# WarmCongee/SDUMC

Hardware: AMD Instinct MI355X
Metric: train samples/sec at MOSEI feature shapes (two-stream forward + 6-term loss + backward + Adam) (higher is better)
Workload: dtype f32

## Files before the change

### sdumc_amd/csrc/attn_pool.hip

```cpp
#include <type_traits>

#include "common.h"
#include "p3_loop.h"
#include <cstring>

namespace {

constexpr int D = SDUMC_D;
constexpr int MAXQ = 8;
constexpr int CH = 64;

__device__ __forceinline__ f32x4 ld4(const float* p) { return *reinterpret_cast<const f32x4*>(p); }
__device__ __forceinline__ void st4(float* p, f32x4 v) { *reinterpret_cast<f32x4*>(p) = v; }
__device__ __forceinline__ void stf_dev(float* p, float v) { __hip_atomic_store(p, v, __ATOMIC_RELAXED, __HIP_MEMORY_SCOPE_AGENT); }
__device__ __forceinline__ float ldf_dev(const float* p) { return __hip_atomic_load(p, __ATOMIC_RELAXED, __HIP_MEMORY_SCOPE_AGENT); }
__device__ __forceinline__ void st4_dev(float* p, f32x4 v) {
#pragma unroll
  for (int j = 0; j < 4; ++j) stf_dev(p + j, v[j]);
}
__device__ __forceinline__ f32x4 ld4_dev(const float* p) {
  f32x4 v;
#pragma unroll
  for (int j = 0; j < 4; ++j) v[j] = ldf_dev(p + j);
  return v;
// ... 1284 lines not shown
    }
  };

  constexpr int nk = D / BK;
#pragma unroll
  for (int s = 0; s < NST - 1; ++s) issue(s);
  int buf = 0, ibuf = NST - 1;
  for (int t = 0; t < nk; ++t) {
    if (t + NST - 2 < nk) __builtin_amdgcn_s_waitcnt(waitcnt_vm((NST - 2) * PER));
    else __builtin_amdgcn_s_waitcnt(waitcnt_vm(0));
    __builtin_amdgcn_s_barrier();
    if (t + NST - 1 < nk) issue(ibuf);
    if constexpr (SPLIT) compute_split(lds + buf * STAGE_BYTES);
    else compute(lds + buf * STAGE_BYTES);
    buf = buf + 1 == NST ? 0 : buf + 1;
    ibuf = ibuf + 1 == NST ? 0 : ibuf + 1;
  }
  __syncthreads();

  float* K_s = reinterpret_cast<float*>(lds);
  float* q_s = reinterpret_cast<float*>(lds + TOP_BYTES);
  float* keys_out = const_cast<float*>(p.keys);
#pragma unroll
  for (int i = 0; i < 2; ++i)
#pragma unroll
    for (int j = 0; j < 2; ++j) {
      const int col = wn0 + 32 * j + li;
      const float bv = u.b_in[col];
#pragma unroll
      for (int e = 0; e < 16; ++e) {
        const int row = 32 * i + (e & 3) + 8 * (e >> 2) + 4 * lh;
        const float kv = fast_tanh(acc[i][j][e] + bv);
        K_s[row * UMCA_LDK + col] = kv;
        if (keys_out && t0 + row < T) keys_out[((size_t)v * T + t0 + row) * D + col] = kv;
      }
    }
  __syncthreads();
  attn_fwd_partial_body<false, 1, false, true>(p, static_cast<float*>(p.workspace), nchunk, chunk, v, K_s, q_s, K_s);
#endif
}
template <bool MASK>
__global__ __launch_bounds__(256, 2) void umca_fwd_kernel(const sdumc_umca u, const int nchunk) {
  extern __shared__ __attribute__((aligned(16))) char lds[];
  umca_fwd_body<MASK, false>(u, nchunk, lds);
}
template <bool MASK>
__global__ __launch_bounds__(256, 2) void umca_fwd_split_kernel(const sdumc_umca u, const int nchunk) {
  extern __shared__ __attribute__((aligned(16))) char lds[];
  umca_fwd_body<MASK, true>(u, nchunk, lds);
}

using K3P3Cfg_m = sdumc_p3::PCfg<64, 4, true, 4>;
using K3P3Cfg_n = sdumc_p3::PCfg<64, 4, false, 4>;
static_assert(K3P3Cfg_m::LDS_BYTES <= TOP_BYTES, "the P3 ring lies inside the key tile's memory");
template <bool MASK>
__global__ __launch_bounds__(256, 2) void umca_fwd_p3_kernel(const sdumc_umca u, const int nchunk) {
#if defined(__HIP_DEVICE_COMPILE__)
  using CF = std::conditional_t<MASK, K3P3Cfg_m, K3P3Cfg_n>;
  extern __shared__ __attribute__((aligned(16))) char lds[];
  const sdumc_attnpool& p = u.a;
  const int tid = threadIdx.x, lane = tid & 63;
  const int wave = __builtin_amdgcn_readfirstlane(tid >> 6);
  const int li = lane & 31, lh = lane >> 5;
  const int wn0 = wave * 64;
  const int chunk = blockIdx.x, v = blockIdx.y;
  const int T = p.T, t0 = chunk * CH, vx = v % p.x_samples;
  const __amdgpu_buffer_rsrc_t ra = __builtin_amdgcn_make_buffer_rsrc(const_cast<void*>(u.x_p3), 0,
      (int)min((size_t)p.x_samples * T * D * 6, (size_t)0xFFFFFFF0u), 0x00020000);
  const uint32_t qw = (p.x_drop.width + 3u) >> 2;
  const __amdgpu_buffer_rsrc_t rbits = __builtin_amdgcn_make_buffer_rsrc(const_cast<uint8_t*>(MASK ? p.x_drop.bits : static_cast<const uint8_t*>(u.x_p3)), 0,
      MASK ? (int)min((size_t)p.V * T * qw, (size_t)0xFFFFFFF0u) : 0, 0x00020000);
  f32x16 acc[2][2];
  sdumc_p3::p3_mainloop<CF>(lds, ra, (int64_t)D * 6, [&](int row) { return vx * T + min(t0 + row, T - 1); },
                            rbits, (int)qw, [&](int row) { return v * T + min(t0 + row, T - 1); },
                            static_cast<const char*>(u.w_in_p3f) + (size_t)(wave * 2) * (size_t)((D / 16) * sdumc_p3::FRAG_KT), (size_t)((D / 16) * sdumc_p3::FRAG_KT),
                            0, D / sdumc_p3::BK, acc);
  __syncthreads();
  const float mscale = MASK ? p.x_drop.scale : 1.f;
  float* K_s = reinterpret_cast<float*>(lds);
  float* q_s = reinterpret_cast<float*>(lds + TOP_BYTES);
  float* keys_out = const_cast<float*>(p.keys);
#pragma unroll
  for (int i = 0; i < 2; ++i)
#pragma unroll
    for (int j = 0; j < 2; ++j) {
      const int col = wn0 + 32 * j + li;
      const float bv = u.b_in[col];
#pragma unroll
      for (int e = 0; e < 16; ++e) {
        const int row = 32 * i + (e & 3) + 8 * (e >> 2) + 4 * lh;
        const float kv = fast_tanh(acc[i][j][e] * mscale + bv);
        K_s[row * UMCA_LDK + col] = kv;
        if (keys_out && t0 + row < T) keys_out[((size_t)v * T + t0 + row) * D + col] = kv;
      }
    }
  __syncthreads();
  attn_fwd_partial_body<false, 1, false, true>(p, static_cast<float*>(p.workspace), nchunk, chunk, v, K_s, q_s, K_s);
#endif
}

}

static inline uint32_t qw_of(const sdumc_dropout& d) { return (d.width + 3u) >> 2; }
extern "C" int sdumc_umca_fwd(const sdumc_umca* up, void* stream) {
  if (!up) return SDUMC_EINVAL;
  sdumc_umca u = *up;
  const sdumc_attnpool& p = u.a;
  if (p.V <= 0 || p.T <= 0 || p.nq < 1 || p.nq > MAXQ || p.x_samples <= 0) return SDUMC_EINVAL;
  if ((p.dim != 0 && p.dim != D) || p.bf16 || p.tickets) return SDUMC_EINVAL;
  if (!p.x || !p.q || !p.attn || !p.pooled || !p.out || !u.w_in || !u.b_in) return SDUMC_EINVAL;
  if (p.x_drop.enabled && !p.x_drop.bits) return SDUMC_EINVAL;
  if ((p.T + CH - 1) / CH > 4096) return SDUMC_EINVAL;
  if (!p.workspace || p.workspace_bytes < sdumc_attnpool_fwd_workspace_bytes_dim(p.V, p.T, p.nq, D)) return SDUMC_ENOMEM;
  static sdumc_dev_once attr;
  if (sdumc_once_per_device(attr, [] {
        return sdumc_set_dyn_lds(&sdumc_k3::umca_fwd_kernel<true>, sdumc_k3::LDS_BYTES) && sdumc_set_dyn_lds(&sdumc_k3::umca_fwd_kernel<false>, sdumc_k3::LDS_BYTES) &&
               sdumc_set_dyn_lds(&sdumc_k3::umca_fwd_split_kernel<true>, sdumc_k3::LDS_BYTES) && sdumc_set_dyn_lds(&sdumc_k3::umca_fwd_split_kernel<false>, sdumc_k3::LDS_BYTES);
      }) != SDUMC_OK)
    return SDUMC_ELAUNCH;
  hipStream_t st = as_stream(stream);
  const int nchunk = (p.T + CH - 1) / CH;
  const dim3 grid(nchunk, p.V), blk(256);
  if (u.x_p3 && u.w_in_p3f) {
    if (!sdumc_split_on_(SDUMC_SPLIT_UMCA)) return SDUMC_EINVAL;
    if ((reinterpret_cast<uintptr_t>(u.x_p3) | reinterpret_cast<uintptr_t>(u.w_in_p3f)) & 15) return SDUMC_EINVAL;
    if (p.x_drop.enabled && (qw_of(p.x_drop) & 3)) return SDUMC_EINVAL;
    static sdumc_dev_once attr_p3;
    if (sdumc_once_per_device(attr_p3, [] {
          return sdumc_set_dyn_lds(&sdumc_k3::umca_fwd_p3_kernel<true>, sdumc_k3::LDS_BYTES) && sdumc_set_dyn_lds(&sdumc_k3::umca_fwd_p3_kernel<false>, sdumc_k3::LDS_BYTES);
// ... 23 lines not shown
```

### sdumc_amd/csrc/gemm_p3.hip

```cpp
#include <algorithm>
#include <cstdlib>

#include "p3_loop.h"

namespace sdumc_p3 {

struct Args {
  sdumc_gemm_p3 g;
  int nsplit, kchunk;
};

template <class CF, int MAPPED = 0>
__global__ __launch_bounds__(CF::NTHR, CF::NW == 4 ? 2 : 1) void gemm_p3_nt_kernel(const Args a) {
#if defined(__HIP_DEVICE_COMPILE__)
  constexpr int BM = CF::BM, TM = CF::TM, TN = CF::TN;
  constexpr bool MASK = CF::MASK;
  const sdumc_gemm_p3& g = a.g;
  extern __shared__ __attribute__((aligned(16))) char lds[];
  const int tid = threadIdx.x, lane = tid & 63;
  const int wave = __builtin_amdgcn_readfirstlane(tid >> 6);
  const int li = lane & 31, lh = lane >> 5;
  const int tiles_n = g.N / BN;
  const int tlin = blockIdx.x;
  const int tile_m = tlin / tiles_n, tile_n = tlin - tile_m * tiles_n;
  const int ks = blockIdx.y;
  const int m0 = tile_m * BM, n0 = tile_n * BN;
  const int kbeg = ks * a.kchunk, kend = min(g.K, kbeg + a.kchunk);
  const int nk = (kend - kbeg) / BK;

#if defined(SDUMC_P3_DBG) && (SDUMC_P3_DBG & 8)
  const uint64_t dbg_t0 = __builtin_amdgcn_s_memtime(), dbg_r0 = __builtin_amdgcn_s_memrealtime();
#endif
  const bool second = g.A2 != nullptr && m0 >= g.a2_row0;
  const int arow0 = second ? g.a2_row0 : 0;
  const int a_rows = g.a_row_mod > 0 ? g.a_row_mod : (g.A2 ? (second ? g.M - g.a2_row0 : g.a2_row0) : g.M);
  const __amdgpu_buffer_rsrc_t ra = __builtin_amdgcn_make_buffer_rsrc(const_cast<void*>(second ? g.A2 : g.A), 0, (int)min((size_t)a_rows * (size_t)g.lda, (size_t)0xFFFFFFF0u), 0x00020000);
  [[maybe_unused]] const __amdgpu_buffer_rsrc_t rbits = __builtin_amdgcn_make_buffer_rsrc(const_cast<uint8_t*>(MASK ? g.a_bits : static_cast<const uint8_t*>(g.A)), 0,
                                                                        MASK ? (int)min((size_t)g.M * (size_t)g.bits_qw, (size_t)0xFFFFFFF0u) : 0, 0x00020000);

  f32x16 acc[TM][TN];
  uint64_t dbg_r1 = 0;
  const char* bw = static_cast<const char*>(g.B) + (size_t)(tile_n * 8 + wave * TN) * (size_t)g.ldb;
  if constexpr (MAPPED == 2) {
    const char* abase = static_cast<const char*>(second ? g.A2 : g.A);
    const int32_t* amap = second ? g.a2_map : g.a_map;
    p3_mainloop<CF>(lds, ra, g.lda,
                    [&](int row) -> const char* { return abase + (size_t)amap[min(m0 + row, g.M - 1) - arow0] * (size_t)g.lda; },
                    rbits, g.bits_qw, [&](int row) { return min(m0 + row, g.M - 1); }, bw, (size_t)g.ldb, kbeg, nk, acc, &dbg_r1);
  } else if constexpr (MAPPED == 1) {
    const int32_t* amap = second ? g.a2_map : g.a_map;
    const __amdgpu_buffer_rsrc_t rm = __builtin_amdgcn_make_buffer_rsrc(const_cast<void*>(second ? g.A2 : g.A), 0, (int)min((size_t)g.a_map_rows * (size_t)g.lda, (size_t)0xFFFFFFF0u), 0x00020000);
    p3_mainloop<CF>(lds, rm, g.lda, [&](int row) { return amap[min(m0 + row, g.M - 1) - arow0]; },
                    rbits, g.bits_qw, [&](int row) { return min(m0 + row, g.M - 1); }, bw, (size_t)g.ldb, kbeg, nk, acc, &dbg_r1);
  } else {
    p3_mainloop<CF>(lds, ra, g.lda,
                    [&](int row) { int r = min(m0 + row, g.M - 1) - arow0; if (g.a_row_mod > 0) r %= g.a_row_mod; return r; },
                    rbits, g.bits_qw, [&](int row) { return min(m0 + row, g.M - 1); }, bw, (size_t)g.ldb, kbeg, nk, acc, &dbg_r1);
  }
  (void)dbg_r1;
#if defined(SDUMC_P3_DBG) && (SDUMC_P3_DBG & 8)
  const uint64_t dbg_r2 = __builtin_amdgcn_s_memrealtime();
#endif
  const bool to_slab = a.nsplit > 1;
  const float mscale = MASK ? g.a_scale : 1.f;
  constexpr int LDT = CF::LDT, WCOLS = 32 * TN, CPW = WCOLS / 8;
  float* tw = reinterpret_cast<float*>(lds) + wave * 32 * LDT;
  const int colw = n0 + WCOLS * wave;
  float bv[8];
#pragma unroll
  for (int c = 0; c < 8; ++c) bv[c] = (!to_slab && g.bias) ? g.bias[colw + 8 * (lane & (CPW - 1)) + c] : 0.f;
  __syncthreads();
#pragma unroll
  for (int i = 0; i < TM; ++i) {
#pragma unroll
    for (int j = 0; j < TN; ++j)
#pragma unroll
      for (int e = 0; e < 16; ++e) tw[((e & 3) + 8 * (e >> 2) + 4 * lh) * LDT + 32 * j + li] = acc[i][j][e] * mscale;
    __builtin_amdgcn_s_waitcnt(0xC07F);
#pragma unroll
    for (int u = lane; u < 32 * CPW; u += 64) {
      const int r = u / CPW, cq = u % CPW;
      const int row = m0 + 32 * i + r, col = colw + 8 * cq;
      if (row < g.M) {
        const f32x4 a0 = *reinterpret_cast<const f32x4*>(tw + r * LDT + 8 * cq), a1 = *reinterpret_cast<const f32x4*>(tw + r * LDT + 8 * cq + 4);
        float v[8] = {a0[0], a0[1], a0[2], a0[3], a1[0], a1[1], a1[2], a1[3]};
        if (to_slab) {
          float* dst = g.workspace + ((size_t)ks * g.M + row) * g.N + col;
          *reinterpret_cast<f32x4*>(dst) = a0;
          *reinterpret_cast<f32x4*>(dst + 4) = a1;
        } else {
#pragma unroll
          for (int c = 0; c < 8; ++c) {
            float x = v[c] + bv[c];
            if (g.act == SDUMC_ACT_TANH) x = fast_tanh(x);
            else if (g.act == SDUMC_ACT_RELU) x = fmaxf(x, 0.f);
            v[c] = x;
          }
          if (g.C) {
            float* dst = g.C + (size_t)row * g.ldc + col;
            *reinterpret_cast<f32x4*>(dst) = f32x4{v[0], v[1], v[2], v[3]};
            *reinterpret_cast<f32x4*>(dst + 4) = f32x4{v[4], v[5], v[6], v[7]};
          }
          if (g.C_p3) {
            u32x4 pl[3];
            split8(v, pl);
            char* dst = static_cast<char*>(g.C_p3) + (size_t)row * (size_t)g.ldc_p3 + (size_t)(col >> 3) * 48;
            *reinterpret_cast<u32x4*>(dst) = pl[0];
            *reinterpret_cast<u32x4*>(dst + 16) = pl[1];
            *reinterpret_cast<u32x4*>(dst + 32) = pl[2];
          }
// ... 62 lines not shown
    *reinterpret_cast<u32x4*>(dst + 16) = pl[1];
    *reinterpret_cast<u32x4*>(dst + 32) = pl[2];
  }
}

__global__ __launch_bounds__(256) void p3_split_kernel(const float* __restrict__ src, int64_t ld, char* __restrict__ dst, int64_t ldp, int64_t rows,
                                                       int cols) {
  const int cpr = cols >> 3;
  const int64_t total = rows * cpr;
  for (int64_t u = (int64_t)blockIdx.x * 256 + threadIdx.x; u < total; u += (int64_t)gridDim.x * 256) {
    const int64_t row = u / cpr;
    const int c = (int)(u - row * cpr);
    const float* s = src + row * ld + 8 * c;
    const f32x4 a0 = *reinterpret_cast<const f32x4*>(s), a1 = *reinterpret_cast<const f32x4*>(s + 4);
    const float v[8] = {a0[0], a0[1], a0[2], a0[3], a1[0], a1[1], a1[2], a1[3]};
    u32x4 pl[3];
    split8(v, pl);
    char* d = dst + row * ldp + (int64_t)c * 48;
    *reinterpret_cast<u32x4*>(d) = pl[0];
    *reinterpret_cast<u32x4*>(d + 16) = pl[1];
    *reinterpret_cast<u32x4*>(d + 32) = pl[2];
  }
}
__global__ __launch_bounds__(256) void p3_split_frag_kernel(const float* __restrict__ src, int64_t ld, char* __restrict__ dst, int rows, int cols) {
  const int cpr = cols >> 3;
  const int64_t total = (int64_t)rows * cpr;
  for (int64_t u = (int64_t)blockIdx.x * 256 + threadIdx.x; u < total; u += (int64_t)gridDim.x * 256) {
    const int row = (int)(u / cpr), c = (int)(u - (int64_t)row * cpr);
    const float* sp = src + (int64_t)row * ld + 8 * c;
    const f32x4 a0 = *reinterpret_cast<const f32x4*>(sp), a1 = *reinterpret_cast<const f32x4*>(sp + 4);
    const float v[8] = {a0[0], a0[1], a0[2], a0[3], a1[0], a1[1], a1[2], a1[3]};
    u32x4 pl[3];
    split8(v, pl);
    const int rb = row >> 5, li = row & 31, kt = c >> 1, lh = c & 1;
    char* d = dst + ((int64_t)rb * (cols >> 4) + kt) * FRAG_KT + (lh * 32 + li) * 16;
    *reinterpret_cast<u32x4*>(d) = pl[0];
    *reinterpret_cast<u32x4*>(d + 1024) = pl[1];
    *reinterpret_cast<u32x4*>(d + 2048) = pl[2];
  }
}

struct FragList {
  int64_t src_off[12], dst_off[12];
  int32_t rows[12], cols[12];
};
__global__ __launch_bounds__(256) void p3_split_frag_multi_kernel(const float* __restrict__ P, char* __restrict__ dst, const FragList L) {
  const int i = blockIdx.y;
  const int rows = L.rows[i], cols = L.cols[i], cpr = cols >> 3;
  const float* src = P + L.src_off[i];
  char* out = dst + L.dst_off[i];
  const int64_t total = (int64_t)rows * cpr;
  for (int64_t u = (int64_t)blockIdx.x * 256 + threadIdx.x; u < total; u += (int64_t)gridDim.x * 256) {
    const int row = (int)(u / cpr), c = (int)(u - (int64_t)row * cpr);
    const float* sp = src + (int64_t)row * cols + 8 * c;
    const f32x4 a0 = *reinterpret_cast<const f32x4*>(sp), a1 = *reinterpret_cast<const f32x4*>(sp + 4);
    const float v[8] = {a0[0], a0[1], a0[2], a0[3], a1[0], a1[1], a1[2], a1[3]};
    u32x4 pl[3];
    split8(v, pl);
    const int rb = row >> 5, li = row & 31, kt = c >> 1, lh = c & 1;
    char* d = out + ((int64_t)rb * (cols >> 4) + kt) * FRAG_KT + (lh * 32 + li) * 16;
    *reinterpret_cast<u32x4*>(d) = pl[0];
    *reinterpret_cast<u32x4*>(d + 1024) = pl[1];
    *reinterpret_cast<u32x4*>(d + 2048) = pl[2];
  }
}
__global__ __launch_bounds__(256) void p3_join_kernel(const char* __restrict__ src, int64_t ldp, float* __restrict__ dst, int64_t ld, int64_t rows,
                                                      int cols) {
  const int cpr = cols >> 3;
  const int64_t total = rows * cpr;
  for (int64_t u = (int64_t)blockIdx.x * 256 + threadIdx.x; u < total; u += (int64_t)gridDim.x * 256) {
    const int64_t row = u / cpr;
    const int c = (int)(u - row * cpr);
    const char* s = src + row * ldp + (int64_t)c * 48;
    const u32x4 p0 = *reinterpret_cast<const u32x4*>(s), p1 = *reinterpret_cast<const u32x4*>(s + 16), p2 = *reinterpret_cast<const u32x4*>(s + 32);
    float v[8];
#pragma unroll
    for (int d = 0; d < 4; ++d) {
      v[2 * d] = (__uint_as_float(p0[d] << 16) + __uint_as_float(p1[d] << 16)) + __uint_as_float(p2[d] << 16);
      v[2 * d + 1] = (__uint_as_float(p0[d] & 0xFFFF0000u) + __uint_as_float(p1[d] & 0xFFFF0000u)) + __uint_as_float(p2[d] & 0xFFFF0000u);
    }
    float* o = dst + row * ld + 8 * c;
    *reinterpret_cast<f32x4*>(o) = f32x4{v[0], v[1], v[2], v[3]};
    *reinterpret_cast<f32x4*>(o + 4) = f32x4{v[4], v[5], v[6], v[7]};
  }
}

struct Plan {
  int bm, nsplit, kchunk;
};
inline Plan plan(const sdumc_gemm_p3& g, size_t have) {
  const int forced = g.tile_m ? g.tile_m : 64;
  const int tiles_n = g.N / BN;
  Plan best{64, 1, g.K};
// ... 41 lines not shown
  if (!g || g->M <= 0 || g->N <= 0 || g->K <= 0 || (g->K % (4 * sdumc_p3::BK))) return 0;
  const sdumc_p3::Plan p = sdumc_p3::plan(*g, (size_t)-1);
  return p.nsplit > 1 ? (size_t)p.nsplit * g->M * g->N * sizeof(float) : 0;
}

extern "C" int sdumc_gemm_p3_nt(const sdumc_gemm_p3* gp, void* stream) {
  using namespace sdumc_p3;
  if (!gp) return SDUMC_EINVAL;
  const sdumc_gemm_p3& g = *gp;
  if (g.M <= 0 || g.N <= 0 || g.K <= 0 || (g.N % BN) || (g.K % (4 * BK))) return SDUMC_EINVAL;
  if (!g.A || !g.B || (!g.C && !g.C_p3)) return SDUMC_EINVAL;
  if ((reinterpret_cast<uintptr_t>(g.A) | reinterpret_cast<uintptr_t>(g.B) | reinterpret_cast<uintptr_t>(g.C) | reinterpret_cast<uintptr_t>(g.C_p3)) & 15) return SDUMC_EINVAL;
  if (g.lda < 6 * (int64_t)g.K || (g.lda & 15)) return SDUMC_EINVAL;
  if (g.ldb < (int64_t)(g.K / BK) * FRAG_KT || (g.ldb & 15)) return SDUMC_EINVAL;
  if (g.C && ((g.ldc & 3) || g.ldc < g.N)) return SDUMC_EINVAL;
  if (g.C_p3 && ((g.ldc_p3 & 15) || g.ldc_p3 < 6 * (int64_t)g.N)) return SDUMC_EINVAL;
  if (g.tile_m != 0 && g.tile_m != 64 && g.tile_m != 96 && g.tile_m != 128) return SDUMC_EINVAL;
  if (g.A2 && (g.a_row_mod || g.a2_row0 <= 0 || g.a2_row0 >= g.M || (g.a2_row0 % 64) || (g.tile_m && g.a2_row0 % g.tile_m) || (reinterpret_cast<uintptr_t>(g.A2) & 15))) return SDUMC_EINVAL;
  if (g.act != SDUMC_ACT_NONE && g.act != SDUMC_ACT_TANH && g.act != SDUMC_ACT_RELU) return SDUMC_EINVAL;
  const bool mapped = g.a_map != nullptr;
  if (mapped && (g.a_row_mod || g.a_bits || (g.A2 != nullptr) != (g.a2_map != nullptr))) return SDUMC_EINVAL;
  if (!mapped && g.a2_map) return SDUMC_EINVAL;
  const size_t a_bytes = (size_t)(g.a_row_mod > 0 ? g.a_row_mod : (g.A2 ? std::max(g.a2_row0, g.M - g.a2_row0) : g.M)) * (size_t)g.lda;
  if (!mapped && a_bytes >= 0xFFFFFFF0u) return SDUMC_EINVAL;
  const bool mask = g.a_bits != nullptr;
  if (mask && (g.bits_qw < g.K / 4 || (g.bits_qw & 3) || (reinterpret_cast<uintptr_t>(g.a_bits) & 3) || (size_t)g.M * g.bits_qw >= 0xFFFFFFF0u)) return SDUMC_EINVAL;
  const Plan p = plan(g, g.workspace ? g.workspace_bytes : 0);
  if (p.nsplit > 1 && (!g.workspace || (reinterpret_cast<uintptr_t>(g.workspace) & 15))) return SDUMC_ENOMEM;
  hipStream_t st = as_stream(stream);
  const int tok = sdumc_prof_begin_(mask ? 27 : 26, 2.0 * g.M * (double)g.N * g.K, stream);
  int rc;
  const bool map32 = mapped && g.a_map_rows > 0 && (size_t)g.a_map_rows * (size_t)g.lda < 0xFFFFFFF0u;
  if (mapped && g.tile_m) return SDUMC_EINVAL;
  if (map32) rc = launch<PCfg<64, 4, false, 4>, 1>(g, p, st);
  else if (mapped) rc = launch<PCfg<64, 4, false, 4>, 2>(g, p, st);
  else if (!g.tile_m) {
    rc = mask ? launch<PCfg<64, 4, true, 4>>(g, p, st) : launch<PCfg<64, 4, false, 4>>(g, p, st);
  } else if (mask) {
    rc = p.bm == 128 ? launch<PCfg<128, 4, true>>(g, p, st) : p.bm == 96 ? launch<PCfg<96, 4, true>>(g, p, st) : launch<PCfg<64, 4, true>>(g, p, st);
  } else {
    rc = p.bm == 128 ? launch<PCfg<128, 4, false>>(g, p, st) : p.bm == 96 ? launch<PCfg<96, 4, false>>(g, p, st) : launch<PCfg<64, 4, false>>(g, p, st);
  }
  if (rc != SDUMC_OK) return rc;
  SDUMC_CHECK_LAUNCH();
  sdumc_prof_end_(tok, stream);
  if (p.nsplit > 1) {
    const size_t units = (size_t)g.M * (g.N >> 3);
    hipLaunchKernelGGL(p3_splitk_reduce_kernel, dim3((unsigned)((units + 255) / 256)), dim3(256), 0, st, g, p.nsplit);
    SDUMC_CHECK_LAUNCH();
  }
  return SDUMC_OK;
}

extern "C" int sdumc_p3_split(const float* src, int64_t ld, void* dst, int64_t ld_bytes, int64_t rows, int32_t cols, void* stream) {
  if (!src || !dst || rows <= 0 || cols <= 0 || (cols & 7) || (ld & 3) || ld < cols || (ld_bytes & 15) || ld_bytes < 6 * (int64_t)cols) return SDUMC_EINVAL;
  if ((reinterpret_cast<uintptr_t>(src) | reinterpret_cast<uintptr_t>(dst)) & 15) return SDUMC_EINVAL;
  const int64_t units = rows * (cols >> 3);
  const unsigned blocks = (unsigned)std::min<int64_t>((units + 255) / 256, 256 * 16);
  hipLaunchKernelGGL(sdumc_p3::p3_split_kernel, dim3(blocks), dim3(256), 0, as_stream(stream), src, ld, static_cast<char*>(dst), ld_bytes, rows, (int)cols);
  SDUMC_CHECK_LAUNCH();
  return SDUMC_OK;
}
extern "C" int sdumc_p3_split_frag(const float* src, int64_t ld, void* dst, int32_t rows, int32_t cols, void* stream) {
  if (!src || !dst || rows <= 0 || cols <= 0 || (rows & 31) || (cols & 15) || (ld & 3) || ld < cols) return SDUMC_EINVAL;
  if ((reinterpret_cast<uintptr_t>(src) | reinterpret_cast<uintptr_t>(dst)) & 15) return SDUMC_EINVAL;
  const int64_t units = (int64_t)rows * (cols >> 3);
  const unsigned blocks = (unsigned)std::min<int64_t>((units + 255) / 256, 256 * 16);
  hipLaunchKernelGGL(sdumc_p3::p3_split_frag_kernel, dim3(blocks), dim3(256), 0, as_stream(stream), src, ld, static_cast<char*>(dst), (int)rows, (int)cols);
  SDUMC_CHECK_LAUNCH();
  return SDUMC_OK;
}
extern "C" int sdumc_p3_split_frag_multi_(const float* P, void* dst, const int64_t* src_off, const int64_t* dst_off, const int32_t* rows,
                                          const int32_t* cols, int n, void* stream) {
  if (!P || !dst || n < 1 || n > 12) return SDUMC_EINVAL;
  sdumc_p3::FragList L;
  int64_t most = 0;
  for (int i = 0; i < n; ++i) {
    if ((rows[i] & 31) || (cols[i] & 15) || (src_off[i] & 3) || (dst_off[i] & 15)) return SDUMC_EINVAL;
    L.src_off[i] = src_off[i]; L.dst_off[i] = dst_off[i]; L.rows[i] = rows[i]; L.cols[i] = cols[i];
    most = std::max<int64_t>(most, (int64_t)rows[i] * (cols[i] >> 3));
  }
  const unsigned bx = (unsigned)std::min<int64_t>((most + 255) / 256, 128);
  hipLaunchKernelGGL(sdumc_p3::p3_split_frag_multi_kernel, dim3(bx, n), dim3(256), 0, as_stream(stream), P, static_cast<char*>(dst), L);
  SDUMC_CHECK_LAUNCH();
  return SDUMC_OK;
}
extern "C" int sdumc_p3_join(const void* src, int64_t ld_bytes, float* dst, int64_t ld, int64_t rows, int32_t cols, void* stream) {
  if (!src || !dst || rows <= 0 || cols <= 0 || (cols & 7) || (ld & 3) || ld < cols || (ld_bytes & 15) || ld_bytes < 6 * (int64_t)cols) return SDUMC_EINVAL;
  if ((reinterpret_cast<uintptr_t>(src) | reinterpret_cast<uintptr_t>(dst)) & 15) return SDUMC_EINVAL;
  const int64_t units = rows * (cols >> 3);
  const unsigned blocks = (unsigned)std::min<int64_t>((units + 255) / 256, 256 * 16);
  hipLaunchKernelGGL(sdumc_p3::p3_join_kernel, dim3(blocks), dim3(256), 0, as_stream(stream), static_cast<const char*>(src), ld_bytes, dst, ld, rows, (int)cols);
  SDUMC_CHECK_LAUNCH();
  return SDUMC_OK;
}

__global__ void sdumc_preload_gemm_p3_kernel() {}
extern "C" int sdumc_preload_gemm_p3_(void) {
  hipFuncAttributes a;
  return hipFuncGetAttributes(&a, reinterpret_cast<const void*>(&sdumc_preload_gemm_p3_kernel)) == hipSuccess ? SDUMC_OK : SDUMC_ELAUNCH;
}
```

### sdumc_amd/csrc/p3_loop.h

```cpp
#pragma once
#include <type_traits>

#include "common.h"

namespace sdumc_p3 {

typedef __attribute__((address_space(3))) void lds_void_t;
typedef __attribute__((address_space(1))) const void gbl_void_t;
typedef const __attribute__((address_space(4))) int32_t const_i32_t;
typedef __bf16 bf16x8 __attribute__((ext_vector_type(8)));
typedef __bf16 bf16x2 __attribute__((ext_vector_type(2)));
typedef float f32x2s __attribute__((ext_vector_type(2)));
typedef uint32_t u32x4 __attribute__((ext_vector_type(4)));

constexpr int waitcnt_vm(int n) { return (n & 0xF) | ((n >> 4) << 14) | (0x7 << 4) | (0xF << 8); }

__device__ __forceinline__ float fast_tanh(float x) { return 1.f - 2.f * __frcp_rn(1.f + __expf(2.f * x)); }

__device__ __forceinline__ uint32_t pk(float x, float y) {
  const f32x2s v = {x, y};
  return __builtin_bit_cast(uint32_t, __builtin_convertvector(v, bf16x2));
}
__device__ __forceinline__ void split8(const float (&v)[8], u32x4 (&pl)[3]) {
#pragma unroll
  for (int d = 0; d < 4; ++d) {
    const float x = v[2 * d], y = v[2 * d + 1];
    const uint32_t p0 = pk(x, y);
    const float x1 = x - __uint_as_float(p0 << 16), y1 = y - __uint_as_float(p0 & 0xFFFF0000u);
    const uint32_t p1 = pk(x1, y1);
    const float x2 = x1 - __uint_as_float(p1 << 16), y2 = y1 - __uint_as_float(p1 & 0xFFFF0000u);
    pl[0][d] = p0;
    pl[1][d] = p1;
    pl[2][d] = pk(x2, y2);
  }
}

constexpr int BN = 256, BK = 16, ROWB = 96;
[[maybe_unused]] constexpr int NBS = 4, DB = 3;
constexpr int FRAG_KT = 3 * 1024;

template <int BM_, int NST_, bool MASK_, int NW_ = 8>
struct PCfg {
  static constexpr int BM = BM_, NST = NST_, TM = BM_ / 32, NW = NW_, TN = BN / (32 * NW_), NTHR = 64 * NW_;
  static constexpr bool MASK = MASK_;
  static constexpr int A_BYTES = BM * ROWB;
  static constexpr int A_P = A_BYTES / 1024;
  static constexpr int NA = (A_P + NW - 1) / NW;
  static constexpr int BITS_BYTES = BM * 4;
  static constexpr int BITS_P = (BITS_BYTES + 255) / 256;
  static constexpr int BITS_LDS = MASK ? BITS_P * 256 : 0;
  static constexpr int STAGE = A_BYTES + BITS_LDS;
  static constexpr int LDT = 32 * TN + 4;
  static constexpr int EPI_BYTES = NW * 32 * LDT * 4;
  static constexpr int LDS_BYTES = NST * STAGE > EPI_BYTES ? NST * STAGE : EPI_BYTES;
  static_assert(BM % 32 == 0 && A_BYTES % 1024 == 0 && NA <= 2 && (NW == 4 || NW == 8), "tile shape");
  static_assert(BITS_P <= NW, "one keep-bits piece per wave");
  static_assert(NST >= DB + 1, "the A stage a step needs must be older in the queue than the B fragments it needs");
  static_assert(3 * (3 * TN + NA + 1) < 64, "vmcnt is a 6-bit counter");
};

template <class CF, class SrcRow, class BitsRow>
__device__ __forceinline__ void p3_mainloop(char* lds, const __amdgpu_buffer_rsrc_t ra, const int64_t lda, SrcRow src_row,
                                            const __amdgpu_buffer_rsrc_t rbits, const int bits_qw, BitsRow bits_row, const char* bwave,
                                            const size_t bblk, const int kbeg, const int nk, f32x16 (&acc)[CF::TM][CF::TN],
                                            uint64_t* stamp = nullptr) {
#if defined(__HIP_DEVICE_COMPILE__)
  constexpr int NST = CF::NST, TM = CF::TM, TN = CF::TN, NW = CF::NW;
  constexpr bool MASK = CF::MASK;
  const int tid = threadIdx.x, lane = tid & 63;
  const int wave = __builtin_amdgcn_readfirstlane(tid >> 6);
  const int li = lane & 31, lh = lane >> 5;
  constexpr bool GA = std::is_pointer<decltype(src_row(0))>::value;
  [[maybe_unused]] uint32_t voff[CF::NA];
  [[maybe_unused]] const char* gaddr[CF::NA];
  bool pvalid[CF::NA];
#pragma unroll
  for (int i = 0; i < CF::NA; ++i) {
    const int piece = wave + i * NW;
    pvalid[i] = piece < CF::A_P;
    const int q = (min(piece, CF::A_P - 1) << 6) + lane;
    const int row = q / 6, sl = q - 6 * row;
    const int hp = sl >= 3 ? 1 : 0, p = sl - 3 * hp;
    const int h = hp ^ ((row >> 3) & 1);
    if constexpr (GA) gaddr[i] = reinterpret_cast<const char*>(src_row(row)) + (size_t)((kbeg >> 3) + h) * 48u + (size_t)p * 16u;
    else voff[i] = (uint32_t)src_row(row) * (uint32_t)lda + (uint32_t)((kbeg >> 3) + h) * 48u + (uint32_t)p * 16u;
  }
  const bool has_bits = MASK && wave < CF::BITS_P;
  uint32_t bvoff = 0;
  if constexpr (MASK) bvoff = (uint32_t)bits_row((wave << 6) + lane) * (uint32_t)bits_qw + (uint32_t)(kbeg >> 2);
  int per = 3 * TN;
#pragma unroll
  for (int i = 0; i < CF::NA; ++i) per += pvalid[i] ? 1 : 0;
  per += has_bits ? 1 : 0;
  auto issue_a = [&](int buf) {
    char* base = lds + buf * CF::STAGE;
#pragma unroll
    for (int i = 0; i < CF::NA; ++i) {
#ifndef SDUMC_P3_DBG
#define SDUMC_P3_DBG 0
#endif
      if (pvalid[i] && !(SDUMC_P3_DBG & 1)) {
        if constexpr (GA) {
          __builtin_amdgcn_global_load_lds((gbl_void_t*)gaddr[i], (lds_void_t*)(base + (wave + i * NW) * 1024), 16, 0, 0);
          gaddr[i] += ROWB;
        } else {
          __builtin_amdgcn_raw_ptr_buffer_load_lds(ra, (lds_void_t*)(base + (wave + i * NW) * 1024), 16, voff[i], 0, 0, 0);
          voff[i] += ROWB;
        }
      }
    }
    if constexpr (MASK) {
      if (has_bits) {
        __builtin_amdgcn_raw_ptr_buffer_load_lds(rbits, (lds_void_t*)(base + CF::A_BYTES + wave * 256), 4, bvoff, 0, 0, 0);
        bvoff += BK / 4;
      }
    }
  };
  auto wait_groups = [&](auto groups_c) {
    constexpr int G = decltype(groups_c)::value, B0 = 3 * TN;
    if (per == B0) __builtin_amdgcn_s_waitcnt(waitcnt_vm(G * B0));
    else if (per == B0 + 1) __builtin_amdgcn_s_waitcnt(waitcnt_vm(G * (B0 + 1)));
    else if (per == B0 + 2) __builtin_amdgcn_s_waitcnt(waitcnt_vm(G * (B0 + 2)));
    else __builtin_amdgcn_s_waitcnt(waitcnt_vm(G * (B0 + 3)));
  };

  const char* bptr = bwave + (size_t)(kbeg >> 4) * FRAG_KT + lane * 16;
  u32x4 pb[NBS][TN][3];
  auto load_b = [&](auto set_c) {
    constexpr int S = decltype(set_c)::value;
#pragma unroll
    for (int j = 0; j < TN; ++j)
#pragma unroll
      for (int p = 0; p < 3; ++p)
        if (!(SDUMC_P3_DBG & 2)) pb[S][j][p] = *reinterpret_cast<const u32x4*>(bptr + j * bblk + p * 1024);
    bptr += FRAG_KT;
  };

#pragma unroll
  for (int i = 0; i < TM; ++i)
#pragma unroll
    for (int j = 0; j < TN; ++j)
#pragma unroll
      for (int e = 0; e < 16; ++e) acc[i][j][e] = 0.f;

  const int lane_off = li * ROWB + ((lh ^ ((li >> 3) & 1)) * 48);
  auto op = [](const u32x4& v) { return __builtin_bit_cast(bf16x8, v); };
  u32x4 pa[2][TM][3];
  uint32_t kb[2][TM];
  auto load_a = [&](const char* base, auto par) {
    constexpr int P = decltype(par)::value;
#pragma unroll
    for (int i = 0; i < TM; ++i) pa[P][i][2] = *reinterpret_cast<const u32x4*>(base + i * 32 * ROWB + lane_off + 32);
#pragma unroll
    for (int i = 0; i < TM; ++i) pa[P][i][0] = *reinterpret_cast<const u32x4*>(base + i * 32 * ROWB + lane_off);
#pragma unroll
    for (int i = 0; i < TM; ++i) pa[P][i][1] = *reinterpret_cast<const u32x4*>(base + i * 32 * ROWB + lane_off + 16);
    if constexpr (MASK) {
#pragma unroll
      for (int i = 0; i < TM; ++i) kb[P][i] = *reinterpret_cast<const uint16_t*>(base + CF::A_BYTES + (32 * i + li) * 4 + 2 * lh);
    }
  };
  auto mfmas = [&](auto par, auto set_c) {
    constexpr int P = decltype(par)::value, S = decltype(set_c)::value;
    if constexpr (MASK) {
#pragma unroll
      for (int i = 0; i < TM; ++i) {
        const uint32_t u = kb[P][i];
        const uint32_t b8 = (u & 0xFu) | ((u >> 4) & 0xF0u);
#pragma unroll
        for (int d = 0; d < 4; ++d) {
          const uint32_t lo = 0u - ((b8 >> (2 * d)) & 1u), hi = 0u - ((b8 >> (2 * d + 1)) & 1u);
          const uint32_t m = (lo & 0xFFFFu) | (hi << 16);
          pa[P][i][0][d] &= m;
          pa[P][i][1][d] &= m;
          pa[P][i][2][d] &= m;
        }
      }
    }
    constexpr int TA[6] = {2, 0, 1, 1, 0, 0}, TB[6] = {0, 2, 1, 0, 1, 0};
#pragma unroll
    for (int t = 0; t < 6; ++t)
#pragma unroll
      for (int i = 0; i < TM; ++i)
#pragma unroll
        for (int j = 0; j < TN; ++j) {
          if (SDUMC_P3_DBG & 4) acc[i][j][t] += __uint_as_float(pa[P][i][TA[t]][0] ^ pb[S][j][TB[t]][1]);
          else acc[i][j] = __builtin_amdgcn_mfma_f32_32x32x16_bf16(op(pa[P][i][TA[t]]), op(pb[S][j][TB[t]]), acc[i][j], 0, 0, 0);
        }
  };
  auto interleave = [&]() {
#pragma unroll
    for (int u = 0; u < 6 * TM * TN; ++u) {
      __builtin_amdgcn_sched_group_barrier(0x008, 1, 0);
      __builtin_amdgcn_sched_group_barrier(0x100, 1, 0);
      __builtin_amdgcn_sched_group_barrier(0x020, 1, 0);
    }
  };

  static_assert(NST >= 4 && DB == 3 && NBS == 4, "the prologue and the unrolled steps are written for these depths");
#pragma unroll
  for (int s0 = 0; s0 <= NST - 4; ++s0) issue_a(s0);
  issue_a(NST - 3);
  load_b(std::integral_constant<int, 0>{});
  issue_a(NST - 2);
  load_b(std::integral_constant<int, 1>{});
  issue_a(NST - 1);
  load_b(std::integral_constant<int, 2>{});
  if constexpr (NST > 4) __builtin_amdgcn_s_waitcnt(waitcnt_vm(0));
  wait_groups(std::integral_constant<int, 3>{});
  __builtin_amdgcn_s_barrier();
  if (stamp) *stamp = __builtin_amdgcn_s_memrealtime();
  load_a(lds, std::integral_constant<int, 0>{});
  int nbuf = 1;
  auto step = [&](int t, auto par, auto set_c, auto steady_c) {
    constexpr int P = decltype(par)::value, S = decltype(set_c)::value;
    constexpr bool STEADY = decltype(steady_c)::value;
    const bool more = STEADY || t + 1 < nk;
    if (STEADY) wait_groups(std::integral_constant<int, DB - 1>{});
    else __builtin_amdgcn_s_waitcnt(waitcnt_vm(0));
    if (more) {
      __builtin_amdgcn_s_waitcnt(0xC07F);
      __builtin_amdgcn_s_barrier();
      if (STEADY || t + NST < nk) issue_a(nbuf == 0 ? NST - 1 : nbuf - 1);
      if (STEADY || t + DB < nk) load_b(std::integral_constant<int, (S + DB) % NBS>{});
      load_a(lds + nbuf * CF::STAGE, std::integral_constant<int, P ^ 1>{});
      nbuf = nbuf + 1 == NST ? 0 : nbuf + 1;
    }
    mfmas(par, set_c);
    if (STEADY) interleave();
  };
  int t = 0;
  for (; t + 3 + NST < nk; t += 4) {
    step(t, std::integral_constant<int, 0>{}, std::integral_constant<int, 0>{}, std::true_type{});
    step(t + 1, std::integral_constant<int, 1>{}, std::integral_constant<int, 1>{}, std::true_type{});
    step(t + 2, std::integral_constant<int, 0>{}, std::integral_constant<int, 2>{}, std::true_type{});
    step(t + 3, std::integral_constant<int, 1>{}, std::integral_constant<int, 3>{}, std::true_type{});
  }
  for (; t < nk; t += 4) {
    step(t, std::integral_constant<int, 0>{}, std::integral_constant<int, 0>{}, std::false_type{});
    step(t + 1, std::integral_constant<int, 1>{}, std::integral_constant<int, 1>{}, std::false_type{});
    step(t + 2, std::integral_constant<int, 0>{}, std::integral_constant<int, 2>{}, std::false_type{});
    step(t + 3, std::integral_constant<int, 1>{}, std::integral_constant<int, 3>{}, std::false_type{});
  }

#endif
}

}
```

Baseline: 50830.

## Add optional 16x16x32 MFMA mainloop and coalesce key tile stores via LDS

Adds a compile-time SHAPE16 variant of the P3 bf16x3 GEMM mainloop using 16x16x32 MFMA with a new weight fragment order, deeper stage ring and 32-k steps, threaded through gemm and UMCA epilogues. Separately, the UMCA forward kernels now write the keys output as row-wise vector stores from the LDS key tile after the barrier, instead of scattered scalar stores per accumulator element. The MFMA shape variant is off unless the build macro is set; the store change adds an LDS read pass but replaces uncoalesced global writes.

```diff
diff --git a/sdumc_amd/csrc/attn_pool.hip b/sdumc_amd/csrc/attn_pool.hip
--- a/sdumc_amd/csrc/attn_pool.hip
+++ b/sdumc_amd/csrc/attn_pool.hip
@@ -1340,10 +1340,14 @@
         const int row = 32 * i + (e & 3) + 8 * (e >> 2) + 4 * lh;
         const float kv = fast_tanh(acc[i][j][e] + bv);
         K_s[row * UMCA_LDK + col] = kv;
-        if (keys_out && t0 + row < T) keys_out[((size_t)v * T + t0 + row) * D + col] = kv;
       }
     }
   __syncthreads();
+  if (keys_out) {
+#pragma unroll 4
+    for (int row = wave; row < CH; row += 4)
+      if (t0 + row < T) *reinterpret_cast<f32x4*>(keys_out + ((size_t)v * T + t0 + row) * D + 4 * lane) = *reinterpret_cast<const f32x4*>(K_s + row * UMCA_LDK + 4 * lane);
+  }
   attn_fwd_partial_body<false, 1, false, true>(p, static_cast<float*>(p.workspace), nchunk, chunk, v, K_s, q_s, K_s);
 #endif
 }
@@ -1358,8 +1362,8 @@
   umca_fwd_body<MASK, true>(u, nchunk, lds);
 }
 
-using K3P3Cfg_m = sdumc_p3::PCfg<64, 4, true, 4>;
-using K3P3Cfg_n = sdumc_p3::PCfg<64, 4, false, 4>;
+using K3P3Cfg_m = sdumc_p3::PCfg<64, sdumc_p3::P3_NST, true, 4>;
+using K3P3Cfg_n = sdumc_p3::PCfg<64, sdumc_p3::P3_NST, false, 4>;
 static_assert(K3P3Cfg_m::LDS_BYTES <= TOP_BYTES, "the P3 ring lies inside the key tile's memory");
 template <bool MASK>
 __global__ __launch_bounds__(256, 2) void umca_fwd_p3_kernel(const sdumc_umca u, const int nchunk) {
@@ -1369,7 +1373,7 @@
   const sdumc_attnpool& p = u.a;
   const int tid = threadIdx.x, lane = tid & 63;
   const int wave = __builtin_amdgcn_readfirstlane(tid >> 6);
-  const int li = lane & 31, lh = lane >> 5;
+  [[maybe_unused]] const int lh = lane >> 5;
   const int wn0 = wave * 64;
   const int chunk = blockIdx.x, v = blockIdx.y;
   const int T = p.T, t0 = chunk * CH, vx = v % p.x_samples;
@@ -1378,7 +1382,7 @@
   const uint32_t qw = (p.x_drop.width + 3u) >> 2;
   const __amdgpu_buffer_rsrc_t rbits = __builtin_amdgcn_make_buffer_rsrc(const_cast<uint8_t*>(MASK ? p.x_drop.bits : static_cast<const uint8_t*>(u.x_p3)), 0,
       MASK ? (int)min((size_t)p.V * T * qw, (size_t)0xFFFFFFF0u) : 0, 0x00020000);
-  f32x16 acc[2][2];
+  typename CF::Acc acc[CF::AM][CF::AN];
   sdumc_p3::p3_mainloop<CF>(lds, ra, (int64_t)D * 6, [&](int row) { return vx * T + min(t0 + row, T - 1); },
                             rbits, (int)qw, [&](int row) { return v * T + min(t0 + row, T - 1); },
                             static_cast<const char*>(u.w_in_p3f) + (size_t)(wave * 2) * (size_t)((D / 16) * sdumc_p3::FRAG_KT), (size_t)((D / 16) * sdumc_p3::FRAG_KT),
@@ -1388,21 +1392,26 @@
   float* K_s = reinterpret_cast<float*>(lds);
   float* q_s = reinterpret_cast<float*>(lds + TOP_BYTES);
   float* keys_out = const_cast<float*>(p.keys);
-#pragma unroll
-  for (int i = 0; i < 2; ++i)
-#pragma unroll
-    for (int j = 0; j < 2; ++j) {
-      const int col = wn0 + 32 * j + li;
+  constexpr int TR = CF::SHAPE16 ? 16 : 32;
+#pragma unroll
+  for (int i = 0; i < CF::AM; ++i)
+#pragma unroll
+    for (int j = 0; j < CF::AN; ++j) {
+      const int col = wn0 + TR * j + (lane & (TR - 1));
       const float bv = u.b_in[col];
 #pragma unroll
-      for (int e = 0; e < 16; ++e) {
-        const int row = 32 * i + (e & 3) + 8 * (e >> 2) + 4 * lh;
+      for (int e = 0; e < (int)(sizeof(typename CF::Acc) / 4); ++e) {
+        const int row = CF::SHAPE16 ? 16 * i + 4 * (lane >> 4) + e : 32 * i + (e & 3) + 8 * (e >> 2) + 4 * lh;
         const float kv = fast_tanh(acc[i][j][e] * mscale + bv);
         K_s[row * UMCA_LDK + col] = kv;
-        if (keys_out && t0 + row < T) keys_out[((size_t)v * T + t0 + row) * D + col] = kv;
       }
     }
   __syncthreads();
+  if (keys_out) {
+#pragma unroll 4
+    for (int row = wave; row < CH; row += 4)
+      if (t0 + row < T) *reinterpret_cast<f32x4*>(keys_out + ((size_t)v * T + t0 + row) * D + 4 * lane) = *reinterpret_cast<const f32x4*>(K_s + row * UMCA_LDK + 4 * lane);
+  }
   attn_fwd_partial_body<false, 1, false, true>(p, static_cast<float*>(p.workspace), nchunk, chunk, v, K_s, q_s, K_s);
 #endif
 }
diff --git a/sdumc_amd/csrc/gemm_p3.hip b/sdumc_amd/csrc/gemm_p3.hip
--- a/sdumc_amd/csrc/gemm_p3.hip
+++ b/sdumc_amd/csrc/gemm_p3.hip
@@ -19,7 +19,7 @@
   extern __shared__ __attribute__((aligned(16))) char lds[];
   const int tid = threadIdx.x, lane = tid & 63;
   const int wave = __builtin_amdgcn_readfirstlane(tid >> 6);
-  const int li = lane & 31, lh = lane >> 5;
+  [[maybe_unused]] const int li = lane & 31, lh = lane >> 5;
   const int tiles_n = g.N / BN;
   const int tlin = blockIdx.x;
   const int tile_m = tlin / tiles_n, tile_n = tlin - tile_m * tiles_n;
@@ -38,7 +38,7 @@
   [[maybe_unused]] const __amdgpu_buffer_rsrc_t rbits = __builtin_amdgcn_make_buffer_rsrc(const_cast<uint8_t*>(MASK ? g.a_bits : static_cast<const uint8_t*>(g.A)), 0,
                                                                         MASK ? (int)min((size_t)g.M * (size_t)g.bits_qw, (size_t)0xFFFFFFF0u) : 0, 0x00020000);
 
-  f32x16 acc[TM][TN];
+  typename CF::Acc acc[CF::AM][CF::AN];
   uint64_t dbg_r1 = 0;
   const char* bw = static_cast<const char*>(g.B) + (size_t)(tile_n * 8 + wave * TN) * (size_t)g.ldb;
   if constexpr (MAPPED == 2) {
@@ -72,10 +72,19 @@
   __syncthreads();
 #pragma unroll
   for (int i = 0; i < TM; ++i) {
-#pragma unroll
-    for (int j = 0; j < TN; ++j)
-#pragma unroll
-      for (int e = 0; e < 16; ++e) tw[((e & 3) + 8 * (e >> 2) + 4 * lh) * LDT + 32 * j + li] = acc[i][j][e] * mscale;
+    if constexpr (CF::SHAPE16) {
+#pragma unroll
+      for (int rb = 0; rb < 2; ++rb)
+#pragma unroll
+        for (int jc = 0; jc < 2 * TN; ++jc)
+#pragma unroll
+          for (int e = 0; e < 4; ++e) tw[(16 * rb + 4 * (lane >> 4) + e) * LDT + 16 * jc + (lane & 15)] = acc[2 * i + rb][jc][e] * mscale;
+    } else {
+#pragma unroll
+      for (int j = 0; j < TN; ++j)
+#pragma unroll
+        for (int e = 0; e < 16; ++e) tw[((e & 3) + 8 * (e >> 2) + 4 * lh) * LDT + 32 * j + li] = acc[i][j][e] * mscale;
+    }
     __builtin_amdgcn_s_waitcnt(0xC07F);
 #pragma unroll
     for (int u = lane; u < 32 * CPW; u += 64) {
@@ -204,8 +213,7 @@
     const float v[8] = {a0[0], a0[1], a0[2], a0[3], a1[0], a1[1], a1[2], a1[3]};
     u32x4 pl[3];
     split8(v, pl);
-    const int rb = row >> 5, li = row & 31, kt = c >> 1, lh = c & 1;
-    char* d = dst + ((int64_t)rb * (cols >> 4) + kt) * FRAG_KT + (lh * 32 + li) * 16;
+    char* d = dst + frag_offset(row, c, cols);
     *reinterpret_cast<u32x4*>(d) = pl[0];
     *reinterpret_cast<u32x4*>(d + 1024) = pl[1];
     *reinterpret_cast<u32x4*>(d + 2048) = pl[2];
@@ -229,8 +237,7 @@
     const float v[8] = {a0[0], a0[1], a0[2], a0[3], a1[0], a1[1], a1[2], a1[3]};
     u32x4 pl[3];
     split8(v, pl);
-    const int rb = row >> 5, li = row & 31, kt = c >> 1, lh = c & 1;
-    char* d = out + ((int64_t)rb * (cols >> 4) + kt) * FRAG_KT + (lh * 32 + li) * 16;
+    char* d = out + frag_offset(row, c, cols);
     *reinterpret_cast<u32x4*>(d) = pl[0];
     *reinterpret_cast<u32x4*>(d + 1024) = pl[1];
     *reinterpret_cast<u32x4*>(d + 2048) = pl[2];
@@ -338,14 +345,14 @@
   int rc;
   const bool map32 = mapped && g.a_map_rows > 0 && (size_t)g.a_map_rows * (size_t)g.lda < 0xFFFFFFF0u;
   if (mapped && g.tile_m) return SDUMC_EINVAL;
-  if (map32) rc = launch<PCfg<64, 4, false, 4>, 1>(g, p, st);
-  else if (mapped) rc = launch<PCfg<64, 4, false, 4>, 2>(g, p, st);
+  if (map32) rc = launch<PCfg<64, P3_NST, false, 4>, 1>(g, p, st);
+  else if (mapped) rc = launch<PCfg<64, P3_NST, false, 4>, 2>(g, p, st);
   else if (!g.tile_m) {
-    rc = mask ? launch<PCfg<64, 4, true, 4>>(g, p, st) : launch<PCfg<64, 4, false, 4>>(g, p, st);
+    rc = mask ? launch<PCfg<64, P3_NST, true, 4>>(g, p, st) : launch<PCfg<64, P3_NST, false, 4>>(g, p, st);
   } else if (mask) {
-    rc = p.bm == 128 ? launch<PCfg<128, 4, true>>(g, p, st) : p.bm == 96 ? launch<PCfg<96, 4, true>>(g, p, st) : launch<PCfg<64, 4, true>>(g, p, st);
+    rc = p.bm == 128 ? launch<PCfg<128, P3_NST, true>>(g, p, st) : p.bm == 96 ? launch<PCfg<96, P3_NST, true>>(g, p, st) : launch<PCfg<64, P3_NST, true>>(g, p, st);
   } else {
-    rc = p.bm == 128 ? launch<PCfg<128, 4, false>>(g, p, st) : p.bm == 96 ? launch<PCfg<96, 4, false>>(g, p, st) : launch<PCfg<64, 4, false>>(g, p, st);
+    rc = p.bm == 128 ? launch<PCfg<128, P3_NST, false>>(g, p, st) : p.bm == 96 ? launch<PCfg<96, P3_NST, false>>(g, p, st) : launch<PCfg<64, P3_NST, false>>(g, p, st);
   }
   if (rc != SDUMC_OK) return rc;
   SDUMC_CHECK_LAUNCH();
@@ -368,7 +375,7 @@
   return SDUMC_OK;
 }
 extern "C" int sdumc_p3_split_frag(const float* src, int64_t ld, void* dst, int32_t rows, int32_t cols, void* stream) {
-  if (!src || !dst || rows <= 0 || cols <= 0 || (rows & 31) || (cols & 15) || (ld & 3) || ld < cols) return SDUMC_EINVAL;
+  if (!src || !dst || rows <= 0 || cols <= 0 || (rows & 31) || (cols % sdumc_p3::FRAG_KMULT) || (ld & 3) || ld < cols) return SDUMC_EINVAL;
   if ((reinterpret_cast<uintptr_t>(src) | reinterpret_cast<uintptr_t>(dst)) & 15) return SDUMC_EINVAL;
   const int64_t units = (int64_t)rows * (cols >> 3);
   const unsigned blocks = (unsigned)std::min<int64_t>((units + 255) / 256, 256 * 16);
@@ -382,7 +389,7 @@
   sdumc_p3::FragList L;
   int64_t most = 0;
   for (int i = 0; i < n; ++i) {
-    if ((rows[i] & 31) || (cols[i] & 15) || (src_off[i] & 3) || (dst_off[i] & 15)) return SDUMC_EINVAL;
+    if ((rows[i] & 31) || (cols[i] % sdumc_p3::FRAG_KMULT) || (src_off[i] & 3) || (dst_off[i] & 15)) return SDUMC_EINVAL;
     L.src_off[i] = src_off[i]; L.dst_off[i] = dst_off[i]; L.rows[i] = rows[i]; L.cols[i] = cols[i];
     most = std::max<int64_t>(most, (int64_t)rows[i] * (cols[i] >> 3));
   }
diff --git a/sdumc_amd/csrc/p3_loop.h b/sdumc_amd/csrc/p3_loop.h
--- a/sdumc_amd/csrc/p3_loop.h
+++ b/sdumc_amd/csrc/p3_loop.h
@@ -1,5 +1,6 @@
 #pragma once
 #include <type_traits>
+#include <utility>
 
 #include "common.h"
 
@@ -36,13 +37,29 @@
 }
 
 constexpr int BN = 256, BK = 16, ROWB = 96;
+#ifndef SDUMC_P3_SHAPE16
+#define SDUMC_P3_SHAPE16 0
+#endif
 [[maybe_unused]] constexpr int NBS = 4, DB = 3;
+constexpr int P3_NST = SDUMC_P3_SHAPE16 ? 6 : 4;
 constexpr int FRAG_KT = 3 * 1024;
 
-template <int BM_, int NST_, bool MASK_, int NW_ = 8>
+__host__ __device__ __forceinline__ int64_t frag_offset(int row, int c, int cols) {
+#if SDUMC_P3_SHAPE16
+  return ((int64_t)(row >> 5) * (cols >> 4) + 2 * (c >> 2) + ((row >> 4) & 1)) * FRAG_KT + (((c & 3) << 4) + (row & 15)) * 16;
+#else
+  return ((int64_t)(row >> 5) * (cols >> 4) + (c >> 1)) * FRAG_KT + (((c & 1) << 5) + (row & 31)) * 16;
+#endif
+}
+constexpr int FRAG_KMULT = SDUMC_P3_SHAPE16 ? 32 : 16;
+
+template <int BM_, int NST_, bool MASK_, int NW_ = 8, bool SHAPE16_ = (SDUMC_P3_SHAPE16 != 0)>
 struct PCfg {
   static constexpr int BM = BM_, NST = NST_, TM = BM_ / 32, NW = NW_, TN = BN / (32 * NW_), NTHR = 64 * NW_;
-  static constexpr bool MASK = MASK_;
+  static constexpr bool MASK = MASK_, SHAPE16 = SHAPE16_;
+  static constexpr int AM = SHAPE16 ? 2 * TM : TM, AN = SHAPE16 ? 2 * TN : TN;
+  using Acc = std::conditional_t<SHAPE16, f32x4, f32x16>;
+  static_assert(SHAPE16_ == (SDUMC_P3_SHAPE16 != 0), "the weight's fragment order is the library's: one shape per build");
   static constexpr int A_BYTES = BM * ROWB;
   static constexpr int A_P = A_BYTES / 1024;
   static constexpr int NA = (A_P + NW - 1) / NW;
@@ -57,19 +74,23 @@
   static_assert(BITS_P <= NW, "one keep-bits piece per wave");
   static_assert(NST >= DB + 1, "the A stage a step needs must be older in the queue than the B fragments it needs");
   static_assert(3 * (3 * TN + NA + 1) < 64, "vmcnt is a 6-bit counter");
+  static_assert(!SHAPE16 || (NST % 2 == 0 && NST >= 4 && (NST / 2 - 1) * 2 * (NA + 1) + 6 * TN < 64 && 4 * (NA + 1) + 6 * TN < 64), "32-k steps: stage pairs; vmcnt is a 6-bit counter");
 };
+
+template <int... I, class F>
+__device__ __forceinline__ void p3_static_for(std::integer_sequence<int, I...>, F&& f) { (f(std::integral_constant<int, I>{}), ...); }
 
 template <class CF, class SrcRow, class BitsRow>
 __device__ __forceinline__ void p3_mainloop(char* lds, const __amdgpu_buffer_rsrc_t ra, const int64_t lda, SrcRow src_row,
                                             const __amdgpu_buffer_rsrc_t rbits, const int bits_qw, BitsRow bits_row, const char* bwave,
-                                            const size_t bblk, const int kbeg, const int nk, f32x16 (&acc)[CF::TM][CF::TN],
+                                            const size_t bblk, const int kbeg, const int nk, typename CF::Acc (&acc)[CF::AM][CF::AN],
                                             uint64_t* stamp = nullptr) {
 #if defined(__HIP_DEVICE_COMPILE__)
   constexpr int NST = CF::NST, TM = CF::TM, TN = CF::TN, NW = CF::NW;
   constexpr bool MASK = CF::MASK;
   const int tid = threadIdx.x, lane = tid & 63;
   const int wave = __builtin_amdgcn_readfirstlane(tid >> 6);
-  const int li = lane & 31, lh = lane >> 5;
+  [[maybe_unused]] const int li = lane & 31, lh = lane >> 5;
   constexpr bool GA = std::is_pointer<decltype(src_row(0))>::value;
   [[maybe_unused]] uint32_t voff[CF::NA];
   [[maybe_unused]] const char* gaddr[CF::NA];
@@ -81,7 +102,7 @@
     const int q = (min(piece, CF::A_P - 1) << 6) + lane;
     const int row = q / 6, sl = q - 6 * row;
     const int hp = sl >= 3 ? 1 : 0, p = sl - 3 * hp;
-    const int h = hp ^ ((row >> 3) & 1);
+    const int h = CF::SHAPE16 ? hp : hp ^ ((row >> 3) & 1);
     if constexpr (GA) gaddr[i] = reinterpret_cast<const char*>(src_row(row)) + (size_t)((kbeg >> 3) + h) * 48u + (size_t)p * 16u;
     else voff[i] = (uint32_t)src_row(row) * (uint32_t)lda + (uint32_t)((kbeg >> 3) + h) * 48u + (uint32_t)p * 16u;
   }
@@ -137,14 +158,137 @@
   };
 
 #pragma unroll
-  for (int i = 0; i < TM; ++i)
-#pragma unroll
-    for (int j = 0; j < TN; ++j)
-#pragma unroll
-      for (int e = 0; e < 16; ++e) acc[i][j][e] = 0.f;
+  for (int i = 0; i < CF::AM; ++i)
+#pragma unroll
+    for (int j = 0; j < CF::AN; ++j)
+#pragma unroll
+      for (int e = 0; e < (int)(sizeof(typename CF::Acc) / 4); ++e) acc[i][j][e] = 0.f;
+  auto op = [](const u32x4& v) { return __builtin_bit_cast(bf16x8, v); };
+  constexpr int TA[6] = {2, 0, 1, 1, 0, 0}, TB[6] = {0, 2, 1, 0, 1, 0};
+  if constexpr (CF::SHAPE16) {
+    constexpr int R = 2 * TM, NS = NST / 2, CN = 2 * TN;
+    const int r16 = lane & 15, kg = lane >> 4;
+    const int lane_off = (kg >> 1) * CF::STAGE + r16 * ROWB + (kg & 1) * 48;
+    [[maybe_unused]] const int bits_off = (kg >> 1) * CF::STAGE + CF::A_BYTES + r16 * 4 + 2 * (kg & 1);
+    const int nsteps = nk >> 1;
+    u32x4 pa[2][3];
+    [[maybe_unused]] uint32_t kb[2];
+    auto load_a = [&](const char* base, auto rb_c) {
+      constexpr int RB = decltype(rb_c)::value, P = RB & 1;
+      const char* s = base + RB * 16 * ROWB + lane_off;
+      pa[P][2] = *reinterpret_cast<const u32x4*>(s + 32);
+      pa[P][0] = *reinterpret_cast<const u32x4*>(s);
+      pa[P][1] = *reinterpret_cast<const u32x4*>(s + 16);
+      if constexpr (MASK) kb[P] = *reinterpret_cast<const uint16_t*>(base + RB * 16 * 4 + bits_off);
+    };
+    auto mfmas = [&](auto rb_c, auto pair_c) {
+      constexpr int RB = decltype(rb_c)::value, P = RB & 1, S0 = 2 * decltype(pair_c)::value;
+      if constexpr (MASK) {
+        const uint32_t u = kb[P];
+        const uint32_t b8 = (u & 0xFu) | ((u >> 4) & 0xF0u);
+#pragma unroll
+        for (int d = 0; d < 4; ++d) {
+          const uint32_t lo = 0u - ((b8 >> (2 * d)) & 1u), hi = 0u - ((b8 >> (2 * d + 1)) & 1u);
+          const uint32_t m = (lo & 0xFFFFu) | (hi << 16);
+          pa[P][0][d] &= m;
+          pa[P][1][d] &= m;
+          pa[P][2][d] &= m;
+        }
+      }
+#pragma unroll
+      for (int t = 0; t < 6; ++t)
+#pragma unroll
+        for (int jc = 0; jc < CN; ++jc) {
+          if (SDUMC_P3_DBG & 4) acc[RB][jc][t & 3] += __uint_as_float(pa[P][TA[t]][0] ^ pb[S0 + (jc & 1)][jc >> 1][TB[t]][1]);
+          else acc[RB][jc] = __builtin_amdgcn_mfma_f32_16x16x32_bf16(op(pa[P][TA[t]]), op(pb[S0 + (jc & 1)][jc >> 1][TB[t]]), acc[RB][jc], 0, 0, 0);
+        }
+    };
+    auto wait_a = [&](auto g_c, auto extra_c) {
+      constexpr int G = decltype(g_c)::value, E = decltype(extra_c)::value;
+      const int q = per - 3 * TN;
+      if (q == 0) __builtin_amdgcn_s_waitcnt(waitcnt_vm(E));
+      else if (q == 1) __builtin_amdgcn_s_waitcnt(waitcnt_vm(2 * G + E));
+      else if (q == 2) __builtin_amdgcn_s_waitcnt(waitcnt_vm(4 * G + E));
+      else __builtin_amdgcn_s_waitcnt(waitcnt_vm(6 * G + E));
+    };
+    static_assert(NS >= 2 && NBS == 4, "two register pairs of B; a ring of at least two steps");
+    using I0 = std::integral_constant<int, 0>;
+    using I1 = std::integral_constant<int, 1>;
+    issue_a(0);
+    issue_a(1);
+    load_b(I0{});
+    load_b(I1{});
+#pragma unroll
+    for (int s0 = 1; s0 <= NS - 2; ++s0) {
+      if (s0 < nsteps) { issue_a(2 * s0); issue_a(2 * s0 + 1); }
+    }
+    load_b(std::integral_constant<int, 2>{});
+    load_b(std::integral_constant<int, 3>{});
+    if (NS - 1 < nsteps) { issue_a(2 * (NS - 1)); issue_a(2 * (NS - 1) + 1); }
+    if (NS <= nsteps) wait_a(std::integral_constant<int, NS - 1>{}, std::integral_constant<int, 6 * TN>{});
+    else __builtin_amdgcn_s_waitcnt(waitcnt_vm(0));
+    __builtin_amdgcn_s_barrier();
+    if (stamp) *stamp = __builtin_amdgcn_s_memrealtime();
+    load_a(lds, I0{});
+    int slot = 0;
+    auto step = [&](int u, auto pair_c, auto steady_c, auto first_c) {
+      constexpr int PAIR = decltype(pair_c)::value;
+      constexpr bool STEADY = decltype(steady_c)::value, FIRST = decltype(first_c)::value;
+      const char* cur = lds + slot * 2 * CF::STAGE;
+      const int nslot = slot + 1 == NS ? 0 : slot + 1, pslot = slot == 0 ? NS - 1 : slot - 1;
+      if constexpr (!FIRST) {
+        if constexpr (!STEADY) __builtin_amdgcn_s_waitcnt(waitcnt_vm(0));
+        if (STEADY || (u > 0 && u + 1 < nsteps)) {
+          load_b(std::integral_constant<int, 2 * (PAIR ^ 1)>{});
+          load_b(std::integral_constant<int, 2 * (PAIR ^ 1) + 1>{});
+        }
+        if (STEADY || (u > 0 && u + NS - 1 < nsteps)) {
+          issue_a(2 * pslot);
+          issue_a(2 * pslot + 1);
+        }
+        if constexpr (STEADY) wait_a(std::integral_constant<int, 2>{}, std::integral_constant<int, 6 * TN>{});
+      }
+      p3_static_for(std::make_integer_sequence<int, R - 1>{}, [&](auto rb_c) {
+        constexpr int RB = decltype(rb_c)::value;
+        load_a(cur, std::integral_constant<int, RB + 1>{});
+        mfmas(rb_c, pair_c);
+        if constexpr (STEADY) {
+#pragma unroll
+          for (int v = 0; v < 6 * CN; ++v) {
+            __builtin_amdgcn_sched_group_barrier(0x008, 1, 0);
+            __builtin_amdgcn_sched_group_barrier(0x100, 1, 0);
+            __builtin_amdgcn_sched_group_barrier(0x020, 1, 0);
+          }
+        }
+      });
+      if (STEADY || u + 1 < nsteps) {
+        if constexpr (STEADY) wait_a(std::integral_constant<int, NS - 2>{}, std::integral_constant<int, (NS > 2 ? 6 * TN : 0)>{});
+        else __builtin_amdgcn_s_waitcnt(waitcnt_vm(0));
+        __builtin_amdgcn_s_waitcnt(0xC07F);
+        __builtin_amdgcn_s_barrier();
+        load_a(lds + nslot * 2 * CF::STAGE, I0{});
+      }
+      mfmas(std::integral_constant<int, R - 1>{}, pair_c);
+      __builtin_amdgcn_sched_barrier(0);
+      slot = nslot;
+    };
+    int u = 0;
+    if (NS < nsteps) {
+      step(0, I0{}, std::true_type{}, std::true_type{});
+      step(1, I1{}, std::true_type{}, std::false_type{});
+      u = 2;
+      for (; u + NS < nsteps; u += 2) {
+        step(u, I0{}, std::true_type{}, std::false_type{});
+        step(u + 1, I1{}, std::true_type{}, std::false_type{});
+      }
+    }
+    for (; u < nsteps; u += 2) {
+      step(u, I0{}, std::false_type{}, std::false_type{});
+      step(u + 1, I1{}, std::false_type{}, std::false_type{});
+    }
+  } else {
 
   const int lane_off = li * ROWB + ((lh ^ ((li >> 3) & 1)) * 48);
-  auto op = [](const u32x4& v) { return __builtin_bit_cast(bf16x8, v); };
   u32x4 pa[2][TM][3];
   uint32_t kb[2][TM];
   auto load_a = [&](const char* base, auto par) {
@@ -177,7 +321,6 @@
         }
       }
     }
-    constexpr int TA[6] = {2, 0, 1, 1, 0, 0}, TB[6] = {0, 2, 1, 0, 1, 0};
 #pragma unroll
     for (int t = 0; t < 6; ++t)
 #pragma unroll
@@ -242,7 +385,7 @@
     step(t + 2, std::integral_constant<int, 0>{}, std::integral_constant<int, 2>{}, std::false_type{});
     step(t + 3, std::integral_constant<int, 1>{}, std::integral_constant<int, 3>{}, std::false_type{});
   }
-
+  }
 #endif
 }
 
```

Result: no change. 51100, median of 6 (+0.5%).
